# ethindp/noise-cpp

Measured on AMD Instinct MI355X. Metric: GiB/s ChaChaPoly AEAD over device-resident 1 KiB Noise records, 1 & 8 GPU, higher is better.
Workload: dtype u32

## Files before the change

### noise-cpp_amd/csrc/aead_kernels.hip

```cpp
#include "chachapoly_device.hpp"
#include "launchers.hpp"
#include "mtile_kernel.hpp"
#include "tile_kernel.hpp"
#include "tile_launch.hpp"

namespace noise_amd {

constexpr int kBlock = 256;

template <bool DECRYPT, bool VEC>
__global__ __launch_bounds__(kBlock) void k_aead_uniform(
    KeyArg key, uint64_t nonce0, const uint8_t *__restrict__ in,
    uint64_t in_stride, uint8_t *out, uint64_t out_stride, uint32_t len,
    const uint8_t *ad, uint64_t ad_stride, uint32_t ad_len, uint8_t *status,
    uint64_t nrec) {
  const uint64_t i = (uint64_t)blockIdx.x * kBlock + threadIdx.x;
  if (i >= nrec) return;
  uint32_t k[8];
#pragma unroll
  for (int j = 0; j < 8; ++j) k[j] = key.w[j];
  const bool ok = aead_record<DECRYPT, VEC>(
      k, nonce0 + i, in + i * in_stride, out + i * out_stride, len,
      ad + i * ad_stride, ad_len);
  if (DECRYPT) status[i] = ok ? 0u : 1u;
// ... 56 lines not shown
  uint4 v = b[0];
  if (sh) {
    const uint4 hi = sh + have > 16u ? b[1] : make_uint4(0u, 0u, 0u, 0u);
    v = extract16(v, hi, sh);
  }
  *reinterpret_cast<uint4 *>(s + i * sstride + 16ull * p) = v;
}

__global__ __launch_bounds__(kBlock) void k_stage_out(const uint8_t *s, uint64_t sstride,
                                                      uint8_t *out, uint64_t out_stride, uint32_t n,
                                                      uint32_t nb, const uint8_t *status,
                                                      int keep_failed, uint64_t nrec) {
  const uint64_t t = (uint64_t)blockIdx.x * kBlock + threadIdx.x;
  const uint64_t i = t / nb;
  const uint32_t bi = (uint32_t)(t % nb);
  if (i >= nrec) return;
  const uintptr_t d = reinterpret_cast<uintptr_t>(out + i * out_stride);
  const uintptr_t blk = (d & ~(uintptr_t)15u) + 16ull * bi;
  const uintptr_t lo = blk > d ? blk : d, hi = blk + 16u < d + n ? blk + 16u : d + n;
  if (lo >= hi) return;
  bool zero = false;
  if (status && status[i] != 0u) {
    if (keep_failed) return;
    zero = true;
  }
  const int64_t off = (int64_t)blk - (int64_t)d;
  const int64_t a0 = off >= 0 ? (off & ~(int64_t)15) : -16;
  const uint32_t sh = (uint32_t)(off - a0);
  const uint8_t *row = s + i * sstride;
  const uint4 z = make_uint4(0u, 0u, 0u, 0u);
  const uint4 A = a0 >= 0 ? *reinterpret_cast<const uint4 *>(row + a0) : z;
  const uint4 B = (sh && a0 + 16 < (int64_t)sstride) ? *reinterpret_cast<const uint4 *>(row + a0 + 16) : z;
  uint4 v = sh ? extract16(A, B, sh) : A;
  if (zero) v = z;
  uint8_t *bp = reinterpret_cast<uint8_t *>(blk);
  if (lo == blk && hi == blk + 16u) {
    store16<true>(bp, v, 16);
  } else {
    const uint32_t w[4] = {v.x, v.y, v.z, v.w};
    for (uint32_t j = (uint32_t)(lo - blk); j < (uint32_t)(hi - blk); ++j)
      bp[j] = (uint8_t)(w[j >> 2] >> (8u * (j & 3u)));
  }
}

#ifndef NOISE_STAGE_BYTES
#define NOISE_STAGE_BYTES (1ull << 30)
#endif
constexpr uint64_t kStageBytes = NOISE_STAGE_BYTES;

#ifndef NOISE_UNIFORM_SPAN
#define NOISE_UNIFORM_SPAN 256
#endif

static hipError_t launch_uniform_exact(bool decrypt, const TileArgs &ta, uint32_t len, bool contig,
                                       hipStream_t stream) {
  for_exact_len(len, [&](auto L) {
    for_bools(decrypt, contig, [&](auto DEC, auto CONTIG) {
      constexpr int LEN = decltype(L)::value;
      hipLaunchKernelGGL((k_aead_tile<decltype(DEC)::value, LEN, decltype(CONTIG)::value, kTileUniform, 0, 1,
                                      (LEN >= 256 && LEN <= 8192) ? NOISE_UNIFORM_SPAN : 256>),
                         tile_grid(ta.nrec), dim3(64), 0, stream, ta);
    });
  });
  return hipGetLastError();
}

static hipError_t launch_uniform_masked(bool decrypt, TileArgs ta, uint32_t len, uint32_t cap,
                                        hipStream_t stream) {
  ta.len = len;
  ta.chunk = -1;
  for_len(MaskedCaps{}, cap, [&](auto L) {
    for_bool(decrypt, [&](auto DEC) {
      constexpr int CAP = decltype(L)::value;
      constexpr uint64_t rps = MTileCfg<CAP>::RPS;
      hipLaunchKernelGGL((k_aead_mtile<decltype(DEC)::value, CAP, kMTUniform>),
                         dim3((unsigned)((ta.nrec + rps - 1) / rps)), dim3(64), 0, stream, ta);
    });
  });
  return hipGetLastError();
}

static hipError_t launch_uniform_staged(bool decrypt, const TileArgs &b, uint32_t len, bool inplace,
                                        hipStream_t stream) {
  const uint64_t nrec = b.nrec;
  const uint64_t sstride = ((uint64_t)len + 31u) & ~15ull;
  const uint64_t per = kStageBytes / sstride > kStageMin ? kStageBytes / sstride : kStageMin;
  const uint64_t cap = nrec < per ? nrec : per;
  void *mem = nullptr;
  hipError_t e = records_scratch_get(&mem, cap * sstride, stream);
  if (e != hipSuccess) return e;
  uint8_t *s = static_cast<uint8_t *>(mem);
  const uint32_t nin = decrypt ? len + 16u : len, nout = decrypt ? len : len + 16u;
  const uint32_t np = (nin + 15u) / 16u, nb = nout / 16u + 2u;
  for (uint64_t r0 = 0; r0 < nrec; r0 += cap) {
    const uint64_t n = nrec - r0 < cap ? nrec - r0 : cap;
    hipLaunchKernelGGL(k_stage_in, grid_for(n * np), dim3(kBlock), 0, stream, b.in + r0 * b.in_stride,
                       b.in_stride, s, sstride, nin, np, n);
    if ((e = hipGetLastError()) != hipSuccess) return e;
    uint8_t *status = b.status ? b.status + r0 : nullptr;
    TileArgs ta = tile_args_strided(s, sstride, s, sstride, status, n);
    ta.key = b.key;
    ta.nonce0 = b.nonce0 + r0;
    e = exact_index(len) >= 0 ? launch_uniform_exact(decrypt, ta, len, false, stream)
                              : launch_uniform_masked(decrypt, ta, len, ceil_capacity(MaskedCaps{}, len), stream);
    if (e != hipSuccess) return e;
    hipLaunchKernelGGL(k_stage_out, grid_for(n * nb), dim3(kBlock), 0, stream, s, sstride,
                       b.out + r0 * b.out_stride, b.out_stride, nout, nb, decrypt ? status : nullptr,
                       inplace ? 1 : 0, n);
    if ((e = hipGetLastError()) != hipSuccess) return e;
  }
  return hipSuccess;
}

hipError_t launch_aead_uniform(bool decrypt, const uint32_t key[8],
                               uint64_t nonce0, const uint8_t *in,
                               uint64_t in_stride, uint8_t *out,
                               uint64_t out_stride, uint32_t len,
                               const uint8_t *ad, uint64_t ad_stride,
                               uint32_t ad_len, uint8_t *status, uint64_t nrec,
                               hipStream_t stream) {
  if (nrec == 0) return hipSuccess;
  KeyArg k;
  for (int j = 0; j < 8; ++j) k.w[j] = key[j];
  const uint64_t align_bits =
      reinterpret_cast<uintptr_t>(in) | reinterpret_cast<uintptr_t>(out) | in_stride | out_stride;
  const bool inplace = in == out && in_stride == out_stride;
  const bool disjoint = in + in_stride * nrec <= out || out + out_stride * nrec <= in;
  const UniformPath path = uniform_path(decrypt, len, ad_len, align_bits, nrec, inplace, disjoint);
  TileArgs ta = tile_args_strided(in, in_stride, out, out_stride, status, nrec);
// ... 48 lines not shown
```

### noise-cpp_amd/csrc/chachapoly_device.hpp

```cpp
#pragma once
#include <hip/hip_runtime.h>
#include <stdint.h>

namespace noise_amd {

struct KeyArg {
  uint32_t w[8];
};

constexpr uint32_t kSigma0 = 0x61707865u, kSigma1 = 0x3320646eu,
                   kSigma2 = 0x79622d32u, kSigma3 = 0x6b206574u;

__device__ __forceinline__ uint32_t rotl32(uint32_t x, int n) {
  return __builtin_amdgcn_alignbit(x, x, 32 - n);
}

#define NOISE_QR(a, b, c, d)              \
  a += b; d = rotl32(d ^ a, 16);          \
  c += d; b = rotl32(b ^ c, 12);          \
  a += b; d = rotl32(d ^ a, 8);           \
  c += d; b = rotl32(b ^ c, 7);

template <int N>
__device__ __forceinline__ uint32_t quad_rot(uint32_t x) {
// ... 17 lines not shown
    d = quad_rot<3>(d);
    NOISE_QR(a, b, c, d)
    b = quad_rot<3>(b);
    c = quad_rot<2>(c);
    d = quad_rot<1>(d);
  }
  out[0] = a + a0;
  out[1] = b + b0;
  out[2] = c + c0;
  out[3] = d + d0;
}

__device__ __forceinline__ void chacha20_block(const uint32_t k[8],
                                               uint32_t ctr, uint32_t n_lo,
                                               uint32_t n_hi, uint32_t ks[16]) {
  uint32_t x0 = kSigma0, x1 = kSigma1, x2 = kSigma2, x3 = kSigma3;
  uint32_t x4 = k[0], x5 = k[1], x6 = k[2], x7 = k[3];
  uint32_t x8 = k[4], x9 = k[5], x10 = k[6], x11 = k[7];
  uint32_t x12 = ctr, x13 = 0, x14 = n_lo, x15 = n_hi;
#pragma unroll
  for (int i = 0; i < 10; ++i) {
    NOISE_QR(x0, x4, x8, x12)
    NOISE_QR(x1, x5, x9, x13)
    NOISE_QR(x2, x6, x10, x14)
    NOISE_QR(x3, x7, x11, x15)
    NOISE_QR(x0, x5, x10, x15)
    NOISE_QR(x1, x6, x11, x12)
    NOISE_QR(x2, x7, x8, x13)
    NOISE_QR(x3, x4, x9, x14)
  }
  ks[0] = x0 + kSigma0;  ks[1] = x1 + kSigma1;
  ks[2] = x2 + kSigma2;  ks[3] = x3 + kSigma3;
  ks[4] = x4 + k[0];     ks[5] = x5 + k[1];
  ks[6] = x6 + k[2];     ks[7] = x7 + k[3];
  ks[8] = x8 + k[4];     ks[9] = x9 + k[5];
  ks[10] = x10 + k[6];   ks[11] = x11 + k[7];
  ks[12] = x12 + ctr;    ks[13] = x13;
  ks[14] = x14 + n_lo;   ks[15] = x15 + n_hi;
}

struct ChaPre {
  uint32_t x1, x5, x9, x13, x2, x6, x10, x14, x3, x7, x11, x15;
};

__device__ __forceinline__ ChaPre chacha_pre(const uint32_t k[8], uint32_t n_lo,
                                             uint32_t n_hi) {
  ChaPre p;
  p.x1 = kSigma1; p.x5 = k[1]; p.x9 = k[5]; p.x13 = 0u;
  p.x2 = kSigma2; p.x6 = k[2]; p.x10 = k[6]; p.x14 = n_lo;
  p.x3 = kSigma3; p.x7 = k[3]; p.x11 = k[7]; p.x15 = n_hi;
  NOISE_QR(p.x1, p.x5, p.x9, p.x13)
  NOISE_QR(p.x2, p.x6, p.x10, p.x14)
  NOISE_QR(p.x3, p.x7, p.x11, p.x15)
  return p;
}

__device__ __forceinline__ void chacha20_block_pre(const uint32_t k[8],
                                                   uint32_t ctr,
                                                   const ChaPre &pre,
                                                   uint32_t n_lo, uint32_t n_hi,
                                                   uint32_t ks[16]) {
  uint32_t x0 = kSigma0, x1 = pre.x1, x2 = pre.x2, x3 = pre.x3;
  uint32_t x4 = k[0], x5 = pre.x5, x6 = pre.x6, x7 = pre.x7;
  uint32_t x8 = k[4], x9 = pre.x9, x10 = pre.x10, x11 = pre.x11;
  uint32_t x12 = ctr, x13 = pre.x13, x14 = pre.x14, x15 = pre.x15;
  NOISE_QR(x0, x4, x8, x12)
  NOISE_QR(x0, x5, x10, x15)
  NOISE_QR(x1, x6, x11, x12)
  NOISE_QR(x2, x7, x8, x13)
  NOISE_QR(x3, x4, x9, x14)
#pragma unroll
  for (int i = 1; i < 10; ++i) {
    NOISE_QR(x0, x4, x8, x12)
    NOISE_QR(x1, x5, x9, x13)
    NOISE_QR(x2, x6, x10, x14)
    NOISE_QR(x3, x7, x11, x15)
    NOISE_QR(x0, x5, x10, x15)
    NOISE_QR(x1, x6, x11, x12)
    NOISE_QR(x2, x7, x8, x13)
    NOISE_QR(x3, x4, x9, x14)
  }
  ks[0] = x0 + kSigma0;  ks[1] = x1 + kSigma1;
  ks[2] = x2 + kSigma2;  ks[3] = x3 + kSigma3;
  ks[4] = x4 + k[0];     ks[5] = x5 + k[1];
  ks[6] = x6 + k[2];     ks[7] = x7 + k[3];
  ks[8] = x8 + k[4];     ks[9] = x9 + k[5];
  ks[10] = x10 + k[6];   ks[11] = x11 + k[7];
  ks[12] = x12 + ctr;    ks[13] = x13;
  ks[14] = x14 + n_lo;   ks[15] = x15 + n_hi;
}

struct Poly1305 {
  uint32_t h0, h1, h2, h3, h4;
  uint32_t r0, r1, r2, r3;
  uint32_t rr0, rr1, rr2, rr3;
  uint32_t r0lo;
  uint32_t s0, s1, s2, s3;
};

__device__ __forceinline__ void poly_init(Poly1305 &p, const uint32_t otk[16]) {
  p.r0 = otk[0] & 0x0fffffffu;
  p.r1 = otk[1] & 0x0ffffffcu;
  p.r2 = otk[2] & 0x0ffffffcu;
  p.r3 = otk[3] & 0x0ffffffcu;
  p.rr0 = (p.r0 >> 2) * 5u;
  p.rr1 = p.r1 + (p.r1 >> 2);
// ... 301 lines not shown
```

### noise-cpp_amd/csrc/records_kernels.hip

```cpp
#include "chachapoly_device.hpp"
#include "launchers.hpp"
#include "mtile_kernel.hpp"
#include "tile_kernel.hpp"
#include "tile_launch.hpp"

namespace noise_amd {

constexpr int kGenBlock = 256;
#ifndef NOISE_CHUNK_W
#define NOISE_CHUNK_W 4
#endif
constexpr unsigned long long kChunkW = NOISE_CHUNK_W;
#ifndef NOISE_CHUNK_MIN
#define NOISE_CHUNK_MIN 65536
#endif
constexpr uint64_t kChunkMinRecords = NOISE_CHUNK_MIN;
constexpr int kHdrWords = kSegChunks <= 4 ? 128 : 256;
#ifndef NOISE_FIN_W
#define NOISE_FIN_W 4
#endif
#ifndef NOISE_XOR_SPAN
#define NOISE_XOR_SPAN 128
#endif
#ifndef NOISE_POLY_SPAN
#define NOISE_POLY_SPAN 256
#endif
#ifndef NOISE_CLS_WAVES
#define NOISE_CLS_WAVES 4096
#endif
#ifndef NOISE_CLS_MIN_CHUNK
#define NOISE_CLS_MIN_CHUNK 256
#endif
constexpr uint32_t kClsWaves = NOISE_CLS_WAVES;
constexpr uint64_t kClsMinChunk = NOISE_CLS_MIN_CHUNK;
static_assert(kClsWaves % 64 == 0 && kClsMinChunk % 64 == 0, "classifier geometry");
#ifndef NOISE_CLASSIFY_MIN
#define NOISE_CLASSIFY_MIN 2048
#endif
constexpr uint64_t kClassifyMin = NOISE_CLASSIFY_MIN;
constexpr uint64_t kClassifyAvgLen = 2048;
#ifndef NOISE_SEG_CAP
#define NOISE_SEG_CAP (1ull << 24)
#endif
constexpr uint64_t kSegCapMax = NOISE_SEG_CAP;
#ifndef NOISE_GRID_CAP
#define NOISE_GRID_CAP 8192u
#endif

__device__ __forceinline__ bool key_row_zero(const uint8_t *keys, uint32_t ki) {
  const uint4 *kp = reinterpret_cast<const uint4 *>(keys + 32ull * ki);
  const uint4 a = kp[0], b = kp[1];
  return (a.x | a.y | a.z | a.w | b.x | b.y | b.z | b.w) == 0u;
}

__device__ __forceinline__ int record_class(const noise_gpu_record &d, const uint8_t *keys,
                                            uint32_t nkeys, const uint8_t *in,
                                            const uint8_t *out) {
  if (d.key_idx >= nkeys || d.ad_len != 0 || d.len == 0) return kClsGeneric;
  if (key_row_zero(keys, d.key_idx)) return kClsGeneric;
  if (((reinterpret_cast<uintptr_t>(in + d.in_off) |
        reinterpret_cast<uintptr_t>(out + d.out_off)) & 15u) != 0)
    return kClsGeneric;
  return len_class(d.len);
}

struct RecHdr {
  unsigned long long counts[kCols];
  unsigned long long cls_base[kCols];
  unsigned long long nlong;
  unsigned long long nseg;
  unsigned long long spare0;
  unsigned long long qsplit[kSegChunks + 1], ssplit[kSegChunks + 1], tsplit[kSegChunks + 1];
  unsigned long long pad[kHdrWords - 3 - 2 * kCols - 3 * (kSegChunks + 1)];
};
static_assert(sizeof(RecHdr) == 8 * kHdrWords, "scratch header layout");

__device__ __forceinline__ int fin_bucket(uint32_t nf) {
  const int b = 31 - __builtin_clz(nf | 1u);
  return b < kFinBuckets - 1 ? b : kFinBuckets - 1;
}

__device__ __forceinline__ uint32_t wave_incl_scan(uint32_t v, uint32_t lane) {
#pragma unroll
  for (int d = 1; d < 64; d <<= 1) {
    const uint32_t t = (uint32_t)__shfl((int)v, (int)(lane >= (uint32_t)d ? lane - d : lane));
    if (lane >= (uint32_t)d) v += t;
  }
  return v;
}

__device__ __forceinline__ unsigned long long wave_incl_scan64(unsigned long long v,
                                                               uint32_t lane) {
#pragma unroll
  for (int d = 1; d < 64; d <<= 1) {
    const int src = (int)(lane >= (uint32_t)d ? lane - d : lane);
    const uint32_t lo = (uint32_t)__shfl((int)(uint32_t)v, src);
    const uint32_t hi = (uint32_t)__shfl((int)(uint32_t)(v >> 32), src);
    if (lane >= (uint32_t)d) v += ((unsigned long long)hi << 32) | lo;
  }
  return v;
// ... 377 lines not shown
      const uint8_t *tp = in + R.in_off + len;
      const uint4 want = (len & 15u) == 0 ? load16<true>(tp, 16) : load16<false>(tp, 16);
      const uint32_t diff = (want.x ^ tag[0]) | (want.y ^ tag[1]) | (want.z ^ tag[2]) |
                            (want.w ^ tag[3]);
      status[R.di] = diff == 0u ? NOISE_GPU_REC_OK : NOISE_GPU_REC_BAD_MAC;
      R.ok = diff == 0u ? 1u : 0u;
    }
  }
}

template <bool DECRYPT>
__global__ __launch_bounds__(kGenBlock) void k_aead_records(
    const uint8_t *__restrict__ keys, uint32_t nkeys,
    const noise_gpu_record *__restrict__ recs, uint64_t nrec,
    const uint32_t *__restrict__ idx, const RecHdr *hdr,
    const uint8_t *in, uint8_t *out, const uint8_t *ad, uint8_t *status) {
  uint64_t base = 0, n = nrec, base2 = 0, n2 = 0;
  if (idx) {
    base = hdr->cls_base[kClsGeneric];
    n = hdr->counts[kClsGeneric];
    base2 = hdr->cls_base[kClsLong] + hdr->nlong;
    n2 = hdr->counts[kClsLong] - hdr->nlong;
  }
#pragma unroll 1
  for (uint64_t i = (uint64_t)blockIdx.x * kGenBlock + threadIdx.x; i < n + n2;
       i += (uint64_t)gridDim.x * kGenBlock) {
    const uint64_t di = idx ? idx[i < n ? base + i : base2 + (i - n)] : i;
    const noise_gpu_record r = recs[di];
    if (r.key_idx >= nkeys) {
      if (DECRYPT) status[di] = NOISE_GPU_REC_BAD_KEY;
      continue;
    }
    const uint4 *kp = reinterpret_cast<const uint4 *>(keys + 32ull * r.key_idx);
    const uint4 ka = kp[0], kb = kp[1];
    const uint32_t k[8] = {ka.x, ka.y, ka.z, ka.w, kb.x, kb.y, kb.z, kb.w};
    if ((ka.x | ka.y | ka.z | ka.w | kb.x | kb.y | kb.z | kb.w) == 0u) {
      if (DECRYPT) status[di] = NOISE_GPU_REC_BAD_KEY;
      continue;
    }
    const uint8_t *src = in + r.in_off;
    uint8_t *dst = out + r.out_off;
    const bool vec = ((reinterpret_cast<uintptr_t>(src) |
                       reinterpret_cast<uintptr_t>(dst) | r.len) & 15u) == 0;
    bool ok;
    if (vec)
      ok = aead_record<DECRYPT, true>(k, r.nonce, src, dst, r.len, ad + r.ad_off, r.ad_len);
    else
      ok = aead_record<DECRYPT, false>(k, r.nonce, src, dst, r.len, ad + r.ad_off, r.ad_len);
    if (DECRYPT) status[di] = ok ? NOISE_GPU_REC_OK : NOISE_GPU_REC_BAD_MAC;
  }
}

static inline uint64_t align_up(uint64_t x, uint64_t a) { return (x + a - 1) / a * a; }
static inline unsigned capped(uint64_t want, uint64_t cap) {
  if (want == 0) want = 1;
  return (unsigned)(want < cap ? want : cap);
}

struct RecCall {
  const uint8_t *keys;
  uint32_t nkeys;
  const noise_gpu_record *recs;
  uint64_t nrec;
  const uint8_t *in;
  uint8_t *out;
  const uint8_t *ad;
  uint8_t *status;
  hipStream_t stream;
};

struct RecScratch {
  RecHdr *hdr;
  uint32_t *part;
  unsigned long long *wbase;
  uint32_t *idx;
  uint32_t *tails, *fin;
  SegRec *rt;
  SegEntry *segs;
  SegPartial *partial;
  uint32_t *partial_hi;
  uint64_t segcap;
  uint64_t bytes = 0;

  RecScratch(void *base, uint64_t nrec, uint64_t nw, uint64_t segcap) : segcap(segcap) {
    uint64_t o = 0;
    auto take = [&](auto *&p, uint64_t n) {
      p = reinterpret_cast<std::remove_reference_t<decltype(p)>>(reinterpret_cast<uintptr_t>(base) + o);
      bytes = o + n * sizeof(*p);
      o = align_up(bytes, 256);
    };
    take(hdr, 1);
    take(part, nw * kCols);
    take(wbase, nw * kCols);
    take(idx, nrec);
    take(tails, nrec);
    take(fin, nrec);
    take(rt, nrec);
    take(segs, segcap);
    take(partial, segcap);
    take(partial_hi, segcap);
  }
};

static TileArgs tile_args_desc(const RecCall &c, const RecScratch &s) {
  TileArgs a{};
  a.in = c.in;
  a.out = c.out;
  a.status = c.status;
  a.keys = c.keys;
  a.nkeys = c.nkeys;
// ... 143 lines not shown
```

### noise-cpp_amd/csrc/tile_kernel.hpp

```cpp
#pragma once
#include "chachapoly_device.hpp"

namespace noise_amd {

template <int L, int SPAN = 256>
struct TileCfg {
  static constexpr int G = L >= SPAN ? L / SPAN : 1;
  static constexpr int RPT = 64 / G;
  static constexpr int CPL = (L / 64) / G;
  static constexpr int BPL = 4 * CPL;
  static constexpr int SPR = L / 16;
  static constexpr int REC_SLOTS = RPT * SPR;
  static constexpr int NSLOT = REC_SLOTS + RPT;
  static constexpr int LOG2G = G == 1 ? 0 : G == 2 ? 1 : G == 4 ? 2 : G == 8 ? 3
                              : G == 16 ? 4 : G == 32 ? 5 : 6;
  static constexpr int LOG2BPL = BPL == 4 ? 2 : BPL == 8 ? 3 : BPL == 16 ? 4 : 5;
  static_assert(L % 64 == 0 && 64 % G == 0 && (L < SPAN || L % SPAN == 0), "tile shape");
  static_assert(G == 1 || BPL == 8 || BPL == 16, "span of 128 or 256 bytes");
};

template <int SPAN>
__device__ __forceinline__ uint32_t swz(uint32_t s) {
  if constexpr (SPAN == 128) return s ^ (((s >> 3) ^ (s >> 6)) & 7u);
  else return s ^ ((s >> 4) & 15u);
// ... 23 lines not shown
struct SegRec {
  uint64_t in_off, out_off, nonce, seg0;
  uint32_t k[8];
  uint32_t key_idx, di, len, nfull;
  uint32_t r[4];
  uint32_t s[4];
  uint32_t pwlo[3][4], pwhi[3];
  uint32_t r64[5];
  uint32_t rtail[5];
  uint32_t ptail[5];
  uint32_t ok;
  uint32_t r16t[5];
};
static_assert(sizeof(SegRec) == 256, "SegRec layout");
struct SegEntry {
  uint32_t q, s;
};
struct SegPartial {
  uint32_t h[4];
};

struct TileArgs {
  KeyArg key;
  uint64_t nonce0;
  const uint8_t *in;
  uint64_t in_stride;
  uint8_t *out;
  uint64_t out_stride;
  uint8_t *status;
  uint64_t nrec;
  int in_place;
  uint32_t nkeys;
  const uint8_t *keys;
  const uint32_t *key_idx;
  const uint64_t *nonces;
  const noise_gpu_record *recs;
  const uint32_t *idx;
  const unsigned long long *cls_base;
  const unsigned long long *counts;
  int cls;
  int cls2;
  const SegEntry *segs;
  const SegRec *rt;
  const unsigned long long *seg_split;
  int chunk;
  SegPartial *partial;
  uint32_t *partial_hi;
  const unsigned long long *nseg;
  uint32_t len;
  const uint32_t *tails;
  const unsigned long long *ntails;
  const unsigned long long *tail_split;
  const unsigned long long *nlong;
};

__device__ __forceinline__ void seg_range(const TileArgs &a, uint64_t &base, uint64_t &n) {
  base = 0;
  n = *a.nseg;
  if (a.seg_split) {
    const uint64_t lo = a.seg_split[a.chunk], hi = a.seg_split[a.chunk + 1];
    base = lo < n ? lo : n;
    n = (hi < n ? hi : n) - base;
  }
}

template <int L, bool DECRYPT, bool CONTIG, int MODE, int ABL, int SPAN>
__device__ __forceinline__ void tile_load(lds_u4 *lds3, const uint8_t *in,
                                          uint64_t in_stride, uint64_t rec0,
                                          uint32_t nv, uint32_t lane,
                                          const uint32_t gl[4],
                                          uint32_t t_rpt, uint32_t own_in_lo,
                                          uint32_t own_in_hi) {
  using C = TileCfg<L, SPAN>;
  if (ABL == 1) return;
  constexpr bool TAGGED_IN = DECRYPT && MODE < kTileSeg;
  constexpr int IN_SLOTS = TAGGED_IN ? C::NSLOT : C::REC_SLOTS;
  if (CONTIG) {
    const uint8_t *base = in + rec0 * in_stride;
    if (nv >= (uint32_t)C::RPT) {
#pragma unroll
      for (int q = 0; q < C::REC_SLOTS / 64; ++q) {
        const uint32_t g = 64u * q + glq<SPAN>(gl, q);
        const uint32_t rr = g / C::SPR;
        lds_dma16_s(base, DECRYPT ? 16u * (g + rr) : 16u * g, (lds_void *)(lds3 + 64 * q));
      }
    } else {
#pragma unroll
      for (int q = 0; q < C::REC_SLOTS / 64; ++q) {
        const uint32_t g = 64u * q + glq<SPAN>(gl, q);
        const uint32_t rr = g / C::SPR;
        const uint32_t off = DECRYPT ? 16u * (g + rr) : 16u * g;
        if (rr < nv) lds_dma16_s(base, off, (lds_void *)(lds3 + 64 * q));
      }
    }
    if (TAGGED_IN) {
#pragma unroll
      for (int q = C::REC_SLOTS / 64; q < (C::NSLOT + 63) / 64; ++q) {
        const uint32_t r = 64u * q + lane - C::REC_SLOTS;
        if (r < nv)
          lds_dma16_s(base, 16u * (r * (C::SPR + 1) + C::SPR), (lds_void *)(lds3 + 64 * q));
      }
    }
  } else if (MODE >= kTileSeg) {
    constexpr int KPR = C::SPR / 64;
#pragma unroll
    for (int q = 0; q < C::REC_SLOTS / 64; ++q) {
// ... 32 lines not shown
                             (uint32_t)__shfl((int)own_in_lo, src);
        rec_base = in + off;
      } else {
        rec_base = in + (rec0 + r) * in_stride;
      }
      if (s < (uint32_t)IN_SLOTS && r < nv)
        lds_dma16_v(rec_base + 16u * p, (lds_void *)(lds3 + 64 * q));
    }
  }
}

struct SegMeta {
  uint32_t k[8], r[4];
  uint32_t nlo, nhi, in_lo, in_hi, out_lo, out_hi, cb, ok, inpl, q;
};
template <int MODE, int SPAN>
__device__ __forceinline__ void seg_meta_load(SegMeta &m, const SegRec *rt, const SegEntry e,
                                              bool valid, const uint8_t *in, const uint8_t *out) {
  constexpr bool XOR = MODE != kTileSegPoly, POLY = MODE != kTileSegXor;
#pragma unroll
  for (int i = 0; i < 8; ++i) m.k[i] = 0u;
#pragma unroll
  for (int i = 0; i < 4; ++i) m.r[i] = 0u;
  m.nlo = m.nhi = m.in_lo = m.in_hi = m.out_lo = m.out_hi = m.cb = m.ok = m.inpl = m.q = 0u;
  if (valid) {
    const SegRec &R = rt[e.q];
    m.q = e.q;
    const uint64_t io = R.in_off + 1024ull * e.s, oo = R.out_off + 1024ull * e.s;
    m.in_lo = (uint32_t)io; m.in_hi = (uint32_t)(io >> 32);
    m.out_lo = (uint32_t)oo; m.out_hi = (uint32_t)(oo >> 32);
    if (XOR) {
      m.nlo = (uint32_t)R.nonce; m.nhi = (uint32_t)(R.nonce >> 32);
      m.cb = 16u * e.s;
#pragma unroll
      for (int i = 0; i < 8; ++i) m.k[i] = R.k[i];
    }
    if (POLY) {
#pragma unroll
      for (int i = 0; i < 4; ++i) m.r[i] = R.r[i];
    }
    if (MODE == kTileSegXor) {
      m.ok = R.ok;
      m.inpl = in + R.in_off == out + R.out_off;
    }

  }
}

template <bool DECRYPT, int L, bool CONTIG, int MODE = kTileUniform, int ABL = 0, int NBUF = 1,
          int SPAN = 256>
__global__ __launch_bounds__(64) void k_aead_tile(const TileArgs a) {
  using C = TileCfg<L, SPAN>;
  constexpr bool KEYED = MODE != kTileUniform;
  constexpr bool SEG = MODE >= kTileSeg;
  constexpr bool DO_POLY = MODE != kTileSegXor;
  constexpr bool DO_XOR = MODE != kTileSegPoly;
  static_assert(MODE < kTileSegPoly || DECRYPT, "the split segment passes are decrypt's");
  constexpr int OPR = (DECRYPT || SEG) ? C::SPR : C::SPR + 1;
  constexpr int OUT_SLOTS = C::RPT * OPR;
  constexpr bool RECW = !DECRYPT && !SEG && C::SPR >= 64 &&
                        C::SPR % 64 == 0;
  constexpr int NDATA = C::RPT * C::SPR / 64;
  constexpr int NOUT = RECW ? NDATA + 1 : (OUT_SLOTS + 63) / 64;
  static_assert(!(CONTIG && SEG), "segment tiles are strided");
  static_assert(!SEG || (L == 1024 && (SPAN == 256 || SPAN == 128)),
                "segments are 1 KiB, 256 or 128 B per lane");
  static_assert(!SEG || !DO_POLY || SPAN == 256, "the SegRec holds the 256-B spans' powers");
  static_assert(NBUF == 1 || NBUF == 2, "one or two tile buffers");
  static_assert(MODE != kTileSegPoly || NBUF == 1, "the Poly1305 pass has one tile buffer");
  __shared__ uint4 lds[NBUF * C::NSLOT];
  const uint32_t lane = threadIdx.x;
  const uint8_t *in = a.in;
  uint8_t *out = a.out;
  uint64_t nrec = a.nrec, dbase = 0;
  if (SEG) seg_range(a, dbase, nrec);
  uint32_t k[8];
#pragma unroll
  for (int i = 0; i < 8; ++i) k[i] = a.key.w[i];

  const uint32_t rho = lane / C::G, j = lane % C::G;
  uint32_t gl[4];
#pragma unroll
  for (int i = 0; i < 4; ++i) gl[i] = swz<SPAN>(64u * i + lane) - 64u * i;

  SegMeta nxt;
  SegEntry nxt_e{0u, 0u};
  if (SEG) {
    const uint64_t g = (uint64_t)blockIdx.x * 64 + lane;
    if (g < nrec) nxt_e = a.segs[dbase + g];
    seg_meta_load<MODE, SPAN>(nxt, a.rt, nxt_e, g < nrec, in, out);
  }

  constexpr int RPS = 64;
  constexpr int NTS = RPS / C::RPT;
#pragma unroll 1
  for (uint64_t super0 = (uint64_t)blockIdx.x * RPS; super0 < nrec;
       super0 += (uint64_t)gridDim.x * RPS) {
  uint32_t kr[4], kss[4];
  F26 pw[C::LOG2G > 0 && !SEG ? C::LOG2G : 1];
  uint32_t own_q = 0;
  uint32_t own_k[8], own_nlo = 0, own_nhi = 0;
  uint32_t own_in_lo = 0, own_in_hi = 0, own_out_lo = 0, own_out_hi = 0;
  uint32_t own_cb = 0;
  bool own_bad = false, own_inplace = false;
  uint32_t own_ok = 1u;
  uint64_t seg_nok = 0, seg_inpl = 0;
  const uint64_t next0 = super0 + (uint64_t)gridDim.x * 64;
  if (SEG) {
#pragma unroll
    for (int i = 0; i < 8; ++i) own_k[i] = nxt.k[i];
#pragma unroll
    for (int i = 0; i < 4; ++i) { kr[i] = nxt.r[i]; kss[i] = 0u; }
    own_q = nxt.q;
    own_nlo = nxt.nlo;
    own_nhi = nxt.nhi;
    own_in_lo = nxt.in_lo; own_in_hi = nxt.in_hi;
    own_out_lo = nxt.out_lo; own_out_hi = nxt.out_hi;
    own_cb = nxt.cb;
    own_ok = nxt.ok;
    own_inplace = nxt.inpl != 0u;
    if (MODE == kTileSegXor) {
      seg_nok = __ballot(own_ok == 0u);
      seg_inpl = __ballot(own_inplace);
    }

    const uint64_t left = nrec - super0;
    tile_load<L, DECRYPT, CONTIG, MODE, ABL, SPAN>(
        NOISE_LDS3(lds), in, a.in_stride, super0,
        left < (uint64_t)C::RPT ? (uint32_t)left : C::RPT, lane, gl, 0u,
        own_in_lo, own_in_hi);
    nxt_e = SegEntry{0u, 0u};
    if (next0 + lane < nrec) nxt_e = a.segs[dbase + next0 + lane];
  } else {
    uint64_t n = a.nonce0 + super0 + lane;
    if (KEYED) {
      const uint64_t rec = super0 + lane;
      uint32_t ki = 0;
      n = 0;
      if (rec < nrec && lane < (uint32_t)RPS) {
        ki = __builtin_nontemporal_load(a.key_idx + rec);
        n = __builtin_nontemporal_load(a.nonces + rec);
      }
      own_bad = ki >= a.nkeys;
      if (own_bad) ki = 0;
      const u32x4 *kp = reinterpret_cast<const u32x4 *>(a.keys + 32ull * ki);
      const u32x4 ka = __builtin_nontemporal_load(kp), kb = __builtin_nontemporal_load(kp + 1);
      own_k[0] = ka.x; own_k[1] = ka.y; own_k[2] = ka.z; own_k[3] = ka.w;
      own_k[4] = kb.x; own_k[5] = kb.y; own_k[6] = kb.z; own_k[7] = kb.w;
      own_bad = own_bad || (ka.x | ka.y | ka.z | ka.w | kb.x | kb.y | kb.z | kb.w) == 0u;
      own_nlo = (uint32_t)n;
      own_nhi = (uint32_t)(n >> 32);
    } else {
#pragma unroll
      for (int i = 0; i < 8; ++i) own_k[i] = k[i];
    }
    {
      const uint64_t left = nrec - super0;
      tile_load<L, DECRYPT, CONTIG, MODE, ABL, SPAN>(
          NOISE_LDS3(lds), in, a.in_stride, super0,
          left < (uint64_t)C::RPT ? (uint32_t)left : C::RPT, lane, gl, 0u,
          own_in_lo, own_in_hi);
    }
    uint32_t otk[16];
    chacha20_block(own_k, 0u, (uint32_t)n, (uint32_t)(n >> 32), otk);
    kr[0] = otk[0] & 0x0fffffffu;
    kr[1] = otk[1] & 0x0ffffffcu;
    kr[2] = otk[2] & 0x0ffffffcu;
    kr[3] = otk[3] & 0x0ffffffcu;
    kss[0] = otk[4]; kss[1] = otk[5]; kss[2] = otk[6]; kss[3] = otk[7];
    if (C::G > 1) {
      F26 x = to26(kr[0], kr[1], kr[2], kr[3], 0u);
#pragma unroll
      for (int b = 0; b < C::LOG2BPL; ++b) x = mul26(x, x);
      pw[0] = x;
#pragma unroll
      for (int b = 1; b < C::LOG2G; ++b) pw[b] = mul26(pw[b - 1], pw[b - 1]);
    }
  }
  (void)own_cb;

  bool prev_all = false;
#pragma unroll 1
  for (int t = 0; t < NTS; ++t) {
    const uint64_t rec0 = super0 + (uint64_t)t * C::RPT;
    if (rec0 >= nrec) break;
    const uint32_t nv = (nrec - rec0) < (uint64_t)C::RPT ? (uint32_t)(nrec - rec0) : C::RPT;
    uint4 *lb = lds + ((NBUF == 2 && (t & 1)) ? C::NSLOT : 0);

    if (NBUF == 2 && prev_all) wait_vmcnt<NOUT>();
    else wait_vmem();
    wave_lds_fence();
    if (SEG && t == 0) seg_meta_load<MODE, SPAN>(nxt, a.rt, nxt_e, next0 + lane < nrec, in, out);
    F26 own_pw;
    if (SEG && DO_POLY) {
      const uint32_t qs = (uint32_t)__shfl((int)own_q, (int)((uint32_t)t * C::RPT + rho));
      const uint32_t m = C::G - 1u - j, mi = m ? m - 1u : 0u;
      const SegRec &R = a.rt[qs];
      const uint4 v = *reinterpret_cast<const uint4 *>(R.pwlo[mi]);
      const uint32_t v4 = R.pwhi[mi];
      own_pw.a[0] = m ? v.x : 1u; own_pw.a[1] = m ? v.y : 0u; own_pw.a[2] = m ? v.z : 0u;
      own_pw.a[3] = m ? v.w : 0u; own_pw.a[4] = m ? v4 : 0u;
    }
    if (NBUF == 2 && t + 1 < NTS) {
      const uint64_t nrec0 = rec0 + C::RPT;
      if (nrec0 < nrec) {
        const uint64_t left = nrec - nrec0;
        tile_load<L, DECRYPT, CONTIG, MODE, ABL, SPAN>(
            NOISE_LDS3(lds + ((t & 1) ? 0 : C::NSLOT)), in, a.in_stride, nrec0,
            left < (uint64_t)C::RPT ? (uint32_t)left : C::RPT, lane, gl,
            (uint32_t)(t + 1) * C::RPT, own_in_lo, own_in_hi);
      }
    }

    const uint32_t src = (uint32_t)t * C::RPT + rho;
    Poly1305 p;
    p.h0 = p.h1 = p.h2 = p.h3 = p.h4 = 0;
    if (DO_POLY) {
      p.r0 = __shfl(kr[0], src); p.r1 = __shfl(kr[1], src);
      p.r2 = __shfl(kr[2], src); p.r3 = __shfl(kr[3], src);
      p.rr0 = (p.r0 >> 2) * 5u;
      p.rr1 = p.r1 + (p.r1 >> 2);
      p.rr2 = p.r2 + (p.r2 >> 2);
      p.rr3 = p.r3 + (p.r3 >> 2);
      p.r0lo = p.r0 & 3u;
      p.s0 = __shfl(kss[0], src); p.s1 = __shfl(kss[1], src);
      p.s2 = __shfl(kss[2], src); p.s3 = __shfl(kss[3], src);
    }

    uint32_t n_lo, n_hi;
    bool bad_key = false;
    uint32_t kt[8];
#pragma unroll
    for (int i = 0; i < 8; ++i) kt[i] = !DO_XOR ? 0u : KEYED ? __shfl(own_k[i], src) : k[i];
    if (KEYED && DO_XOR) {
      n_lo = __shfl(own_nlo, src);
      n_hi = __shfl(own_nhi, src);
      bad_key = __shfl((int)own_bad, src) != 0;
    } else if (!KEYED) {
      const uint64_t n = a.nonce0 + rec0 + rho;
      n_lo = (uint32_t)n;
      n_hi = (uint32_t)(n >> 32);
    } else {
      n_lo = n_hi = 0u;
    }
    const uint32_t c0 = j * C::CPL;
    const uint32_t cb = 1u + c0 + (SEG && DO_XOR ? (uint32_t)__shfl((int)own_cb, src) : 0u);
    ChaPre pre{};
    uint32_t ks[16];
    if (DO_XOR) {
      pre = chacha_pre(kt, n_lo, n_hi);
      chacha20_block_pre(kt, cb, pre, n_lo, n_hi, ks);
    }
#pragma unroll
    for (int kk = 0; kk < C::CPL; ++kk) {
      const uint32_t c = c0 + kk;
      uint32_t ksn[16];
      if (DO_XOR && kk + 1 < C::CPL) chacha20_block_pre(kt, cb + 1u + kk, pre, n_lo, n_hi, ksn);
#pragma unroll
      for (int q = 0; q < 4; ++q) {
        const uint32_t slot = swz<SPAN>(rho * C::SPR + 4u * c + q);
        const uint4 v = lb[slot];
        uint4 o = v;
        if (DO_XOR) {
          o.x = v.x ^ ks[4 * q + 0];
          o.y = v.y ^ ks[4 * q + 1];
          o.z = v.z ^ ks[4 * q + 2];
          o.w = v.w ^ ks[4 * q + 3];
          lb[slot] = o;
        }
        if (!DO_POLY) {
        } else if (ABL == 2) { p.h0 ^= o.x ^ v.y; p.h1 ^= o.z ^ v.w; }
        else if (DECRYPT) poly_block(p, v.x, v.y, v.z, v.w);
        else poly_block(p, o.x, o.y, o.z, o.w);
      }
      if (DO_XOR && kk + 1 < C::CPL) {
#pragma unroll
        for (int i = 0; i < 16; ++i) ks[i] = ksn[i];
      }
    }
    if (C::G > 1 && DO_POLY) {
      F26 h = to26(p.h0, p.h1, p.h2, p.h3, p.h4);
      if (SEG) {
        h = mul26(h, own_pw);
      } else {
        const uint32_t m = C::G - 1 - j;
#pragma unroll
        for (int b = 0; b < C::LOG2G; ++b) {
          F26 f;
          const bool use = (m >> b) & 1u;
#pragma unroll
          for (int i = 0; i < 5; ++i) {
            const uint32_t w = __shfl(pw[b].a[i], src);
            f.a[i] = use ? w : (i == 0 ? 1u : 0u);
          }
          h = mul26(h, f);
        }
      }
#pragma unroll
      for (int b = 0; b < C::LOG2G; ++b) {
        if (b == 4) carry26(h);
#pragma unroll
        for (int i = 0; i < 5; ++i) h.a[i] += __shfl_xor(h.a[i], 1 << b);
      }
      carry26(h);
      carry26(h);
      from26(h, p.h0, p.h1, p.h2, p.h3, p.h4);
    }
    uint32_t tag[4] = {0u, 0u, 0u, 0u};
    const bool valid = rho < nv;
    if (SEG) {
      if (DO_POLY && j == 0 && valid) {
        const u32x4 w0 = {p.h0, p.h1, p.h2, p.h3};
        const uint64_t g = dbase + super0 + (uint64_t)t * C::RPT + rho;
        __builtin_nontemporal_store(w0, (g_u32x4 *)(a.partial + g));
        __builtin_nontemporal_store(p.h4, (__attribute__((address_space(1))) uint32_t *)(a.partial_hi + g));
      }
    } else {
      poly_block(p, 0u, 0u, (uint32_t)L, 0u);
      poly_final(p, tag);
    }
    uint64_t fail_mask = 0;
    const uint64_t badk_mask = KEYED ? __ballot(j == 0 && bad_key) : 0ull;
    fail_mask = badk_mask;
    constexpr bool PER_REC_INPL = MODE == kTileSegXor;
    uint64_t inpl_seg = 0;
    if (MODE == kTileSegXor) {
      const uint32_t nok = (uint32_t)(seg_nok >> (t * C::RPT)), ip = (uint32_t)(seg_inpl >> (t * C::RPT));
#pragma unroll
      for (int r = 0; r < C::RPT; ++r) {
        fail_mask |= (uint64_t)((nok >> r) & 1u) << (r * C::G);
        inpl_seg |= (uint64_t)((ip >> r) & 1u) << (r * C::G);
      }
    } else if (SEG) {
    } else if (DECRYPT) {
      const uint4 want = lb[C::REC_SLOTS + rho];
      const uint32_t diff = (want.x ^ tag[0]) | (want.y ^ tag[1]) |
                            (want.z ^ tag[2]) | (want.w ^ tag[3]);
      fail_mask |= __ballot(j == 0 && diff != 0u);
      if (j == 0 && valid) {
        a.status[rec0 + rho] = bad_key ? 2u : (diff ? 1u : 0u);
      }
    } else if (j == 0) {
      lb[C::REC_SLOTS + rho] = make_uint4(tag[0], tag[1], tag[2], tag[3]);
    }
    const uint64_t inpl_mask = MODE == kTileSegXor ? inpl_seg : 0ull;
    wave_lds_fence();
    if (!DO_XOR) {
      prev_all = false;
      if (t + 1 < NTS) {
        const uint64_t nrec0 = rec0 + C::RPT;
        if (nrec0 < nrec) {
          wait_lds();
          wave_lds_fence();
          const uint64_t left = nrec - nrec0;
          tile_load<L, DECRYPT, CONTIG, MODE, ABL, SPAN>(
              NOISE_LDS3(lds), in, a.in_stride, nrec0,
              left < (uint64_t)C::RPT ? (uint32_t)left : C::RPT, lane, gl,
              (uint32_t)(t + 1) * C::RPT, own_in_lo, own_in_hi);
        }
      }
      continue;
    }

    constexpr int NPART = (KEYED && NBUF == 1 && NOUT > 8) ? 2 : 1;
    constexpr int NQ = (NOUT + NPART - 1) / NPART;
    const bool full = nv == (uint32_t)C::RPT;
    constexpr bool RECQ = SEG;
    auto piece = [&](int q, uint32_t &r, uint32_t &pc, uint32_t &slot, bool &ok) {
      if constexpr (RECW) {
        if (q < NDATA) {
          r = (uint32_t)q / (C::SPR / 64);
          pc = 64u * ((uint32_t)q % (C::SPR / 64)) + lane;
          slot = swz<SPAN>(64u * q + lane);
          ok = true;
        } else {
          r = lane < (uint32_t)C::RPT ? lane : 0u;
          pc = C::SPR;
          slot = C::REC_SLOTS + r;
          ok = lane < (uint32_t)C::RPT;
        }
        return;
      }
      if (RECQ) {
        if (q < NDATA) {
          r = (uint32_t)q / (C::SPR / 64);
          pc = 64u * ((uint32_t)q % (C::SPR / 64)) + lane;
          slot = swz<SPAN>(64u * q + lane);
          ok = true;
        } else {
          r = lane < (uint32_t)C::RPT ? lane : 0u; pc = C::SPR; slot = C::REC_SLOTS + r;
          ok = lane < (uint32_t)C::RPT;
        }
        return;
      }
      const uint32_t g = 64u * q + lane;
      r = g / OPR;
      pc = g % OPR;
      if (CONTIG && DECRYPT) slot = 64u * q + glq<SPAN>(gl, q);
      else slot = pc < (uint32_t)C::SPR ? swz<SPAN>(r * C::SPR + pc) : C::REC_SLOTS + r;
      ok = OUT_SLOTS % 64 == 0 || g < (uint32_t)OUT_SLOTS;
    };
#pragma unroll
    for (int part = 0; part < NPART; ++part) {
      const int q0 = part * NQ;
      uint4 ov[NQ];
      bool st[NQ];
#pragma unroll
      for (int qq = 0; qq < NQ; ++qq) {
        const int q = q0 + qq;
        if (q >= NOUT) break;
        uint32_t r, pc, slot;
        bool ok;
        piece(q, r, pc, slot, ok);
        st[qq] = ok && (full || r < nv);
        ov[qq] = lb[slot < (uint32_t)C::NSLOT ? slot : 0u];
      }
      if ((DECRYPT || KEYED) && fail_mask != 0) {
#pragma unroll
        for (int qq = 0; qq < NQ; ++qq) {
          const int q = q0 + qq;
          if (q >= NOUT) break;
          uint32_t r, pc, slot;
          bool ok;
          piece(q, r, pc, slot, ok);
          if ((fail_mask >> (r * C::G)) & 1u) {
            const bool bad_key_rec = KEYED && ((badk_mask >> (r * C::G)) & 1u);
            const bool inpl = PER_REC_INPL ? ((inpl_mask >> (r * C::G)) & 1u) != 0
                                           : a.in_place != 0;
            st[qq] = st[qq] && DECRYPT && !inpl && !bad_key_rec;
            ov[qq] = make_uint4(0u, 0u, 0u, 0u);
          }
        }
      }
      if (part == NPART - 1) {
        wait_lds();
        wave_lds_fence();
        if (NBUF == 1 && t + 1 < NTS) {
          const uint64_t nrec0 = rec0 + C::RPT;
          if (nrec0 < nrec) {
            const uint64_t left = nrec - nrec0;
            tile_load<L, DECRYPT, CONTIG, MODE, ABL, SPAN>(
                NOISE_LDS3(lds), in, a.in_stride, nrec0,
                left < (uint64_t)C::RPT ? (uint32_t)left : C::RPT, lane, gl,
                (uint32_t)(t + 1) * C::RPT, own_in_lo, own_in_hi);
          }
        }
      }
#pragma unroll
      for (int qq = 0; qq < NQ; ++qq) {
        const int q = q0 + qq;
        if (q >= NOUT) break;
        const uint32_t g = 64u * q + lane;
        uint32_t r, pc, slot;
        bool ok;
        piece(q, r, pc, slot, ok);
        bool store = st[qq];
        if (ABL == 1) store = store && (ov[qq].x == 0x12345678u && ov[qq].y == 0x9abcdef0u);
        uint8_t *dst;
        if (RECQ && q < NDATA) {
          const uint32_t kl = (uint32_t)t * C::RPT + (uint32_t)q / (C::SPR / 64);
          const uint64_t off = join64((uint32_t)__builtin_amdgcn_readlane((int)own_out_hi, (int)kl),
                                      (uint32_t)__builtin_amdgcn_readlane((int)own_out_lo, (int)kl));
          dst = out + off + 16u * pc;
        } else {
          dst = out + rec0 * a.out_stride +
                ((CONTIG && !RECW) ? 16ull * g : r * a.out_stride + 16u * pc);
        }
        if (store) store16<true>(dst, ov[qq], 16);
      }
    }
    prev_all = ABL == 0 && full && fail_mask == 0;
  }
  }
}

}
```

### noise-cpp_amd/csrc/tile_launch.hpp

```cpp
#pragma once
#include <type_traits>

#include "tile_classes.hpp"
#include "tile_kernel.hpp"

namespace noise_amd {

inline TileArgs tile_args_strided(const uint8_t *in, uint64_t in_stride, uint8_t *out,
                                  uint64_t out_stride, uint8_t *status, uint64_t nrec) {
  TileArgs ta{};
  ta.in = in;
  ta.in_stride = in_stride;
  ta.out = out;
  ta.out_stride = out_stride;
  ta.status = status;
  ta.nrec = nrec;
  ta.in_place = in == out;
  return ta;
}
inline dim3 tile_grid(uint64_t nrec) { return dim3((unsigned)((nrec + 63) / 64)); }

template <int... L, class F>
bool for_len(LenList<L...>, uint32_t len, F &&f) {
  return ((len == (uint32_t)L && (f(std::integral_constant<int, L>{}), true)) || ...);
}
template <class F>
bool for_exact_len(uint32_t len, F &&f) {
  return for_len(ExactLens{}, len, f);
}
template <class F>
void for_bool(bool a, F &&f) {
  if (a) f(std::true_type{});
  else f(std::false_type{});
}
template <class F>
void for_bools(bool a, bool b, F &&f) {
  for_bool(a, [&](auto A) { for_bool(b, [&](auto B) { f(A, B); }); });
}
template <int FIRST, int LAST, class F>
void for_exact_classes(F &&f) {
  f(std::integral_constant<int, FIRST>{}, std::integral_constant<int, (int)ExactLens::v[FIRST]>{});
  if constexpr (FIRST != LAST) for_exact_classes<FIRST + (FIRST < LAST ? 1 : -1), LAST>(f);
}

}
```

Measured before the change: 1628.

## Precompute nonce-independent ChaCha columns on host and trim Poly1305 combine work

For the uniform-key path, the host now precomputes the first double-round column quarter-rounds that depend only on the key and the high nonce word. Launches are split so the low nonce word never wraps within a run, which lets kernels skip two of the three precomputed column rounds per block. It also folds the Poly1305 lane powers into a single multiply for G=2/4, drops the two carry passes on the non-segmented path, and splits the failed-record output handling into a separate loop copy for long records. It also caps the masked-tile grid. These changes add host-side setup and code size, and rely on mul26 inputs staying in range without the extra carries.

New measurement: 1649 (median of 6 runs). 1.01x the previous value.

```diff
diff --git a/noise-cpp_amd/csrc/aead_kernels.hip b/noise-cpp_amd/csrc/aead_kernels.hip
--- a/noise-cpp_amd/csrc/aead_kernels.hip
+++ b/noise-cpp_amd/csrc/aead_kernels.hip
@@ -132,16 +132,25 @@
 #define NOISE_UNIFORM_SPAN 256
 #endif
 
-static hipError_t launch_uniform_exact(bool decrypt, const TileArgs &ta, uint32_t len, bool contig,
+static hipError_t launch_uniform_exact(bool decrypt, const TileArgs &b, uint32_t len, bool contig,
                                        hipStream_t stream) {
-  for_exact_len(len, [&](auto L) {
-    for_bools(decrypt, contig, [&](auto DEC, auto CONTIG) {
-      constexpr int LEN = decltype(L)::value;
-      hipLaunchKernelGGL((k_aead_tile<decltype(DEC)::value, LEN, decltype(CONTIG)::value, kTileUniform, 0, 1,
-                                      (LEN >= 256 && LEN <= 8192) ? NOISE_UNIFORM_SPAN : 256>),
-                         tile_grid(ta.nrec), dim3(64), 0, stream, ta);
+  for (uint64_t r0 = 0; r0 < b.nrec;) {
+    TileArgs ta = b;
+    tile_set_uniform(ta, b.key, b.nonce0 + r0);
+    ta.nrec = uniform_run_len(ta.nonce0, b.nrec - r0);
+    ta.in = b.in + r0 * b.in_stride;
+    ta.out = b.out + r0 * b.out_stride;
+    if (b.status) ta.status = b.status + r0;
+    for_exact_len(len, [&](auto L) {
+      for_bools(decrypt, contig, [&](auto DEC, auto CONTIG) {
+        constexpr int LEN = decltype(L)::value;
+        hipLaunchKernelGGL((k_aead_tile<decltype(DEC)::value, LEN, decltype(CONTIG)::value, kTileUniform, 0, 1,
+                                        (LEN >= 256 && LEN <= 8192) ? NOISE_UNIFORM_SPAN : 256>),
+                           tile_grid(ta.nrec), dim3(64), 0, stream, ta);
+      });
     });
-  });
+    r0 += ta.nrec;
+  }
   return hipGetLastError();
 }
 
@@ -154,7 +163,7 @@
       constexpr int CAP = decltype(L)::value;
       constexpr uint64_t rps = MTileCfg<CAP>::RPS;
       hipLaunchKernelGGL((k_aead_mtile<decltype(DEC)::value, CAP, kMTUniform>),
-                         dim3((unsigned)((ta.nrec + rps - 1) / rps)), dim3(64), 0, stream, ta);
+                         dim3(capped((ta.nrec + rps - 1) / rps, NOISE_GRID_CAP)), dim3(64), 0, stream, ta);
     });
   });
   return hipGetLastError();
diff --git a/noise-cpp_amd/csrc/chachapoly_device.hpp b/noise-cpp_amd/csrc/chachapoly_device.hpp
--- a/noise-cpp_amd/csrc/chachapoly_device.hpp
+++ b/noise-cpp_amd/csrc/chachapoly_device.hpp
@@ -93,6 +93,20 @@
   NOISE_QR(p.x1, p.x5, p.x9, p.x13)
   NOISE_QR(p.x2, p.x6, p.x10, p.x14)
   NOISE_QR(p.x3, p.x7, p.x11, p.x15)
+  return p;
+}
+
+struct ChaUniform {
+  uint32_t c1[4], c3[4];
+};
+
+__device__ __forceinline__ ChaPre chacha_pre_uniform(const uint32_t k[8], uint32_t n_lo,
+                                                     const ChaUniform &u) {
+  ChaPre p;
+  p.x1 = u.c1[0]; p.x5 = u.c1[1]; p.x9 = u.c1[2]; p.x13 = u.c1[3];
+  p.x2 = kSigma2; p.x6 = k[2]; p.x10 = k[6]; p.x14 = n_lo;
+  p.x3 = u.c3[0]; p.x7 = u.c3[1]; p.x11 = u.c3[2]; p.x15 = u.c3[3];
+  NOISE_QR(p.x2, p.x6, p.x10, p.x14)
   return p;
 }
 
diff --git a/noise-cpp_amd/csrc/records_kernels.hip b/noise-cpp_amd/csrc/records_kernels.hip
--- a/noise-cpp_amd/csrc/records_kernels.hip
+++ b/noise-cpp_amd/csrc/records_kernels.hip
@@ -43,9 +43,6 @@
 #define NOISE_SEG_CAP (1ull << 24)
 #endif
 constexpr uint64_t kSegCapMax = NOISE_SEG_CAP;
-#ifndef NOISE_GRID_CAP
-#define NOISE_GRID_CAP 8192u
-#endif
 
 __device__ __forceinline__ bool key_row_zero(const uint8_t *keys, uint32_t ki) {
   const uint4 *kp = reinterpret_cast<const uint4 *>(keys + 32ull * ki);
@@ -529,10 +526,6 @@
 }
 
 static inline uint64_t align_up(uint64_t x, uint64_t a) { return (x + a - 1) / a * a; }
-static inline unsigned capped(uint64_t want, uint64_t cap) {
-  if (want == 0) want = 1;
-  return (unsigned)(want < cap ? want : cap);
-}
 
 struct RecCall {
   const uint8_t *keys;
diff --git a/noise-cpp_amd/csrc/tile_kernel.hpp b/noise-cpp_amd/csrc/tile_kernel.hpp
--- a/noise-cpp_amd/csrc/tile_kernel.hpp
+++ b/noise-cpp_amd/csrc/tile_kernel.hpp
@@ -99,6 +99,7 @@
   const unsigned long long *ntails;
   const unsigned long long *tail_split;
   const unsigned long long *nlong;
+  ChaUniform uni;
 };
 
 __device__ __forceinline__ void seg_range(const TileArgs &a, uint64_t &base, uint64_t &n) {
@@ -237,6 +238,7 @@
 __global__ __launch_bounds__(64) void k_aead_tile(const TileArgs a) {
   using C = TileCfg<L, SPAN>;
   constexpr bool KEYED = MODE != kTileUniform;
+  constexpr bool UNI_PRE = !KEYED && L >= 128;
   constexpr bool SEG = MODE >= kTileSeg;
   constexpr bool DO_POLY = MODE != kTileSegXor;
   constexpr bool DO_XOR = MODE != kTileSegPoly;
@@ -282,7 +284,9 @@
   for (uint64_t super0 = (uint64_t)blockIdx.x * RPS; super0 < nrec;
        super0 += (uint64_t)gridDim.x * RPS) {
   uint32_t kr[4], kss[4];
-  F26 pw[C::LOG2G > 0 && !SEG ? C::LOG2G : 1];
+  constexpr bool ONE_PROD = !SEG && (C::G == 2 || (C::G == 4 && !KEYED));
+  constexpr int NPW = SEG || C::G == 1 ? 1 : ONE_PROD ? C::G - 1 : C::LOG2G;
+  F26 pw[NPW];
   uint32_t own_q = 0;
   uint32_t own_k[8], own_nlo = 0, own_nhi = 0;
   uint32_t own_in_lo = 0, own_in_hi = 0, own_out_lo = 0, own_out_hi = 0;
@@ -317,7 +321,8 @@
     nxt_e = SegEntry{0u, 0u};
     if (next0 + lane < nrec) nxt_e = a.segs[dbase + next0 + lane];
   } else {
-    uint64_t n = a.nonce0 + super0 + lane;
+    uint64_t n = UNI_PRE ? join64((uint32_t)(a.nonce0 >> 32), (uint32_t)a.nonce0 + (uint32_t)super0 + lane)
+                         : a.nonce0 + super0 + lane;
     if (KEYED) {
       const uint64_t rec = super0 + lane;
       uint32_t ki = 0;
@@ -347,7 +352,12 @@
           own_in_lo, own_in_hi);
     }
     uint32_t otk[16];
-    chacha20_block(own_k, 0u, (uint32_t)n, (uint32_t)(n >> 32), otk);
+    if (!UNI_PRE) {
+      chacha20_block(own_k, 0u, (uint32_t)n, (uint32_t)(n >> 32), otk);
+    } else {
+      const ChaPre kpre = chacha_pre_uniform(own_k, (uint32_t)n, a.uni);
+      chacha20_block_pre(own_k, 0u, kpre, (uint32_t)n, (uint32_t)(n >> 32), otk);
+    }
     kr[0] = otk[0] & 0x0fffffffu;
     kr[1] = otk[1] & 0x0ffffffcu;
     kr[2] = otk[2] & 0x0ffffffcu;
@@ -358,8 +368,15 @@
 #pragma unroll
       for (int b = 0; b < C::LOG2BPL; ++b) x = mul26(x, x);
       pw[0] = x;
-#pragma unroll
-      for (int b = 1; b < C::LOG2G; ++b) pw[b] = mul26(pw[b - 1], pw[b - 1]);
+      if constexpr (ONE_PROD) {
+        if constexpr (C::G == 4) {
+          pw[1] = mul26(pw[0], pw[0]);
+          pw[2] = mul26(pw[1], pw[0]);
+        }
+      } else {
+#pragma unroll
+        for (int b = 1; b < C::LOG2G; ++b) pw[b] = mul26(pw[b - 1], pw[b - 1]);
+      }
     }
   }
   (void)own_cb;
@@ -423,8 +440,8 @@
       bad_key = __shfl((int)own_bad, src) != 0;
     } else if (!KEYED) {
       const uint64_t n = a.nonce0 + rec0 + rho;
-      n_lo = (uint32_t)n;
-      n_hi = (uint32_t)(n >> 32);
+      n_lo = UNI_PRE ? (uint32_t)a.nonce0 + (uint32_t)rec0 + rho : (uint32_t)n;
+      n_hi = UNI_PRE ? (uint32_t)(a.nonce0 >> 32) : (uint32_t)(n >> 32);
     } else {
       n_lo = n_hi = 0u;
     }
@@ -433,7 +450,7 @@
     ChaPre pre{};
     uint32_t ks[16];
     if (DO_XOR) {
-      pre = chacha_pre(kt, n_lo, n_hi);
+      pre = UNI_PRE ? chacha_pre_uniform(kt, n_lo, a.uni) : chacha_pre(kt, n_lo, n_hi);
       chacha20_block_pre(kt, cb, pre, n_lo, n_hi, ks);
     }
 #pragma unroll
@@ -467,6 +484,19 @@
       F26 h = to26(p.h0, p.h1, p.h2, p.h3, p.h4);
       if (SEG) {
         h = mul26(h, own_pw);
+      } else if constexpr (ONE_PROD) {
+        const uint32_t m = C::G - 1 - j;
+        F26 f;
+#pragma unroll
+        for (int i = 0; i < 5; ++i) {
+          uint32_t w = __shfl(pw[0].a[i], src);
+          if constexpr (C::G == 4) {
+            const uint32_t w2 = __shfl(pw[1].a[i], src), w3 = __shfl(pw[2].a[i], src);
+            w = m == 3u ? w3 : m == 2u ? w2 : w;
+          }
+          f.a[i] = m ? w : (i == 0 ? 1u : 0u);
+        }
+        h = mul26(h, f);
       } else {
         const uint32_t m = C::G - 1 - j;
 #pragma unroll
@@ -487,8 +517,10 @@
 #pragma unroll
         for (int i = 0; i < 5; ++i) h.a[i] += __shfl_xor(h.a[i], 1 << b);
       }
-      carry26(h);
-      carry26(h);
+      if (SEG) {
+        carry26(h);
+        carry26(h);
+      }
       from26(h, p.h0, p.h1, p.h2, p.h3, p.h4);
     }
     uint32_t tag[4] = {0u, 0u, 0u, 0u};
@@ -585,6 +617,11 @@
       else slot = pc < (uint32_t)C::SPR ? swz<SPAN>(r * C::SPR + pc) : C::REC_SLOTS + r;
       ok = OUT_SLOTS % 64 == 0 || g < (uint32_t)OUT_SLOTS;
     };
+    constexpr bool SPLIT_FAILED = (DECRYPT || KEYED) && L >= 1024;
+    const bool any_failed = (DECRYPT || KEYED) && fail_mask != 0;
+#pragma unroll
+    for (int copy = 0; copy < (SPLIT_FAILED ? 2 : 1); ++copy) {
+    if (SPLIT_FAILED && any_failed != (copy == 1)) continue;
 #pragma unroll
     for (int part = 0; part < NPART; ++part) {
       const int q0 = part * NQ;
@@ -600,7 +637,7 @@
         st[qq] = ok && (full || r < nv);
         ov[qq] = lb[slot < (uint32_t)C::NSLOT ? slot : 0u];
       }
-      if ((DECRYPT || KEYED) && fail_mask != 0) {
+      if (SPLIT_FAILED ? copy == 1 : any_failed) {
 #pragma unroll
         for (int qq = 0; qq < NQ; ++qq) {
           const int q = q0 + qq;
@@ -654,6 +691,7 @@
         if (store) store16<true>(dst, ov[qq], 16);
       }
     }
+    }
     prev_all = ABL == 0 && full && fail_mask == 0;
   }
   }
diff --git a/noise-cpp_amd/csrc/tile_launch.hpp b/noise-cpp_amd/csrc/tile_launch.hpp
--- a/noise-cpp_amd/csrc/tile_launch.hpp
+++ b/noise-cpp_amd/csrc/tile_launch.hpp
@@ -17,6 +17,36 @@
   ta.nrec = nrec;
   ta.in_place = in == out;
   return ta;
+}
+inline void tile_set_uniform(TileArgs &ta, const KeyArg &key, uint64_t nonce0) {
+  ta.key = key;
+  ta.nonce0 = nonce0;
+  auto rotl = [](uint32_t x, int n) { return (x << n) | (x >> (32 - n)); };
+  auto column = [&](uint32_t x[4]) {
+    x[0] += x[1]; x[3] = rotl(x[3] ^ x[0], 16);
+    x[2] += x[3]; x[1] = rotl(x[1] ^ x[2], 12);
+    x[0] += x[1]; x[3] = rotl(x[3] ^ x[0], 8);
+    x[2] += x[3]; x[1] = rotl(x[1] ^ x[2], 7);
+  };
+  const uint32_t c1[4] = {kSigma1, key.w[1], key.w[5], 0u};
+  const uint32_t c3[4] = {kSigma3, key.w[3], key.w[7], (uint32_t)(nonce0 >> 32)};
+  for (int i = 0; i < 4; ++i) {
+    ta.uni.c1[i] = c1[i];
+    ta.uni.c3[i] = c3[i];
+  }
+  column(ta.uni.c1);
+  column(ta.uni.c3);
+}
+inline uint64_t uniform_run_len(uint64_t nonce0, uint64_t nrec) {
+  const uint64_t room = (1ull << 32) - (nonce0 & 0xffffffffull);
+  return nrec < room ? nrec : room;
+}
+#ifndef NOISE_GRID_CAP
+#define NOISE_GRID_CAP 8192u
+#endif
+inline unsigned capped(uint64_t want, uint64_t cap) {
+  if (want == 0) want = 1;
+  return (unsigned)(want < cap ? want : cap);
 }
 inline dim3 tile_grid(uint64_t nrec) { return dim3((unsigned)((nrec + 63) / 64)); }
 
```
